# dmar-bonn/ipp-rl

Hardware: AMD Instinct MI355X
Metric: env-steps/s (batched) on 50x50 grid (higher is better)
Workload: dtype f32

## Files before the change

ipp-rl_amd/csrc/ipp_common.h:

```cpp
#pragma once
#include <hip/hip_runtime.h>
#include <stdint.h>
#include <type_traits>

#include "../../include/ipp_engine.h"

#include "ipp_instrument.h"

namespace ipp {

constexpr int kWave = 64;
constexpr int kCountSlots = 64;
#ifndef IPP_PREP_THREADS
#define IPP_PREP_THREADS 128
#endif
constexpr int kPrepThreads = IPP_PREP_THREADS;
constexpr int kMaxTileThreads = 640;
constexpr int kBandRows = 20;
constexpr double kSqrt3 = 1.7320508075688772;

struct ItemHdr {
    int env, dst, rank, status;
    int xl, xr, yu, yd;
    int w, h, nx, ny;
// ... 88 lines not shown
    float* mean;
    float* diag;
    float* gt;
    int* gt_slot;
    double* prior;
    int* rank;
    int* colspan;
    int* colrect;
    int rect_meta;
    int patch;
    int pw, ph;
    int pstride;
    int plw;
    int pcap;
    int punits;
    int pos0;
    unsigned long long* counters;
    unsigned long long* item_counts;
    float* cov;
    uint64_t cov_slot;
    ItemHdr* hdr;
    float* linv;
    float* yv;
    float* q;
    float* wc;
    double* partial;
    double* dbg;
    int dbg_capture;
    double* grf_h;
    double2* grf_cs;
// ... 338 lines not shown
```

ipp-rl_amd/csrc/ipp_engine.hip:

```cpp
#include <hip/hip_runtime.h>
#include <hip/hip_ext.h>

#include <algorithm>
#include <cmath>
#include <cstdarg>
#include <cstdio>
#include <cstdlib>
#include <cstring>
#include <new>
#include <string>
#include <vector>

#include "ipp_common.h"
#include "ipp_host.h"
#include "k_gain.h"
#include "k_gain_factor.h"
#include "k_step_factor.h"
#include "k_step_patch.h"
#include "k_gain_wave.h"
#include "k_misc.h"
#include "k_grf_dft.h"
#include "k_grf_hartley.h"
#include "k_grf_fft.h"
#include "k_fields.h"
// ... 70 lines not shown
    size_t tree_step_lds = 0;
    size_t tree_gain_lds = 0;
    hipStream_t side = nullptr;
    hipEvent_t ev_begin = nullptr, ev_end = nullptr;
    hipEvent_t ev_prep[8] = {};
    ProfSlot prof[kProfKinds];
    std::vector<ProfEvent> prof_pending;
    int last_n = 0;
    uint64_t last_needed_bytes = 0;
};

struct Layout {
    int N, Npad, T, n_tiles, win_tiles, MC, FC, QS, q_rows, VEC;
    bool patch;
    PatchGeo pg;
    uint64_t off_mean, off_diag, off_gt, off_gtslot, off_prior, off_rank, off_span, off_cnt, off_icnt, off_cov, off_hdr, off_linv, off_yv, off_q, off_wc,
        off_partial, off_dbg, off_grfh, off_grfcs, off_grfg, off_grfhp, off_grfamp, off_grfraw, off_grfraw2, off_sc_hdr, off_sc_ext, off_sc_mask, off_sc_G, off_sc_P, off_tr_cov, off_tr_diag, off_tr_meta, off_sc_ndiag, total, cov_slot_floats;
};

uint64_t q_item_floats(const Layout& L) {
    const uint64_t lq = ((uint64_t)L.MC * L.MC + L.MC + 3) & ~(uint64_t)3;
    uint64_t q = lq + (uint64_t)(L.q_rows + 8) * L.QS;
    if (L.patch) q = std::max<uint64_t>(q, (uint64_t)L.q_rows * kPatchRec);
    return (q + 15) & ~(uint64_t)15;
}

bool patch_layout(const ipp_config& c, int MC, const Switches& sw) {
    if (c.state_repr != IPP_FACTOR || c.window_rows <= 0 || MC != 9) return false;
    if (c.tile_threads != 0) return false;
    if (c.x_dim % 2 != 0 || c.x_dim > 256 || c.y_dim > 256) return false;
    if (!(c.x_dim > 2 * c.window_rows + 13)) return false;
// ... 89 lines not shown
        const long rows = std::min<long>(c.y_dim, 2L * c.window_rows + 2L * L.MC);
        L.win_tiles = (int)std::min<long>(L.n_tiles, (rows * c.x_dim + 64 * L.VEC - 1) / (64 * L.VEC) + 1);
    }
    L.q_rows = (c.state_repr == IPP_FACTOR) ? c.rank_cap : L.FC;
    L.cov_slot_floats = (c.state_repr == IPP_FACTOR) ? (uint64_t)c.rank_cap * L.Npad : (uint64_t)L.N * L.Npad;
    if (L.patch) L.cov_slot_floats = (uint64_t)c.rank_cap * L.pg.pstride;
    uint64_t o = 0;
    const uint64_t cap = c.capacity, mb = c.max_batch, np = L.Npad;
    L.off_mean = o; o += up(cap * np * 4);
    L.off_diag = o; o += up(cap * np * 4);
    L.off_gt = o; o += up(2 * cap * np * 4);
    L.off_gtslot = o; o += up(2 * cap * 4);
    L.off_prior = o; o += up(cap * 2 * 8);
    L.off_rank = o; o += up(cap * 4);
    L.off_span = o; o += (c.state_repr == IPP_FACTOR) ? up(2 * cap * (uint64_t)c.rank_cap * 4) : 0;
    L.off_cnt = o; o += up((uint64_t)kCountSlots * 128);
    L.off_icnt = o; o += up((uint64_t)c.max_batch * 16);
    L.off_cov = o; o += up(cap * L.cov_slot_floats * 4);
    L.off_hdr = o; o += up(mb * sizeof(ItemHdr));
    L.off_linv = o; o += up(mb * L.MC * L.MC * 4);
    L.off_yv = o; o += up(mb * L.MC * 4);
    L.off_q = o; o += up(mb * q_item_floats(L) * 4 + 4096);
    L.off_wc = o; o += (c.state_repr == IPP_DENSE) ? up(mb * L.MC * np * 4) : 0;
    L.off_partial = o; o += up(mb * L.n_tiles * 8);
    L.off_dbg = o; o += up(mb * (2 * L.MC * L.MC + 2 * L.MC) * 8);
    L.off_grfh = o; o += up((uint64_t)L.N * 8);
    L.off_grfcs = o; o += up((uint64_t)c.x_dim * 16);
    L.off_grfg = o; o += up((uint64_t)(c.y_dim / 2 + 1) * c.x_dim * 8);
    {
        const uint64_t npad = 16 * (uint64_t)((std::max(c.x_dim, c.y_dim) + 15) / 16);
// ... 128 lines not shown
        for (auto& x : iv[k]) {
            if (x.first > end) { p.busy_ms += x.second - x.first; end = x.second; }
            else if (x.second > end) { p.busy_ms += x.second - end; end = x.second; }
        }
        p.busy_launches += (int64_t)iv[k].size();
    }
}

size_t gain_lds_bytes(const View& v, int q_chunk, int lut_cap) {
    const size_t MC = v.meas_cap, QS = v.q_stride;
    size_t b = std::max((size_t)(q_chunk + 2 * kPipe) * QS, (size_t)((lut_cap + 3) & ~3)) * 4 + ((MC * MC + 3) & ~(size_t)3) * 4 + ((MC + 3) & ~(size_t)3) * 4 + 16 * 8;
    b += (size_t)std::max(q_chunk, v.q_rows) * 4;
    return (b + 15) & ~(size_t)15;
}

#define IPP_STEP_PATCH_KERNELS(X)      \
    X(2, kPatchKP, kPatchMinW, 0)      \
    X(3, kPatchKP, kPatchMinW, 0)      \
    X(3, kPatchKP, kPatchMinW, 1)      \
    X(3, kPatchKP, kPatchMinW, 2)      \
    X(2, IPP_PATCH_BIGKP, 6, 0)
#define IPP_TREE_PATCH_KERNELS(X) X(3, 0) X(3, 1)

using StepPatchKernel = decltype(&k_step_patch<3>);
using TreePatchKernel = decltype(&k_tree_patch<3>);
template <bool BUD>
StepPatchKernel patch_kernel(const PatchVariant& pv) {
#define X(NW, KPN, MINW, RJN) \
    if (pv.waves == NW && pv.kpn == KPN && pv.minw == MINW && pv.rjn == RJN) return k_step_patch<NW, KPN, MINW, RJN, BUD>;
    IPP_STEP_PATCH_KERNELS(X)
#undef X
    return nullptr;
}
TreePatchKernel tree_patch_kernel(const PatchVariant& pv) {
#define X(NW, RJN) if (pv.waves == NW && pv.rjn == RJN) return k_tree_patch<NW, RJN>;
    IPP_TREE_PATCH_KERNELS(X)
#undef X
    return nullptr;
}

template <int MC, int VEC>
void launch_chunk(Engine* e, const View& v, const int32_t* env_ids, const int32_t* dst_ids, int n, const double* action,
                  const double* prev, const float* noise, unsigned flags, float* reward, int32_t* status, hipStream_t s,
                  hipEvent_t prep_done, const AutoReset& ar) {
// ... 281 lines not shown
    v.meas_cap = L.MC; v.fp_cap = L.FC; v.q_stride = L.QS; v.q_rows = L.q_rows; v.q_item = q_item_floats(L);
    v.res = cfg->resolution; v.tanx = cfg->tan_half_fov_x; v.tany = cfg->tan_half_fov_y; v.rf_alt = cfg->rf_altitude;
    v.coeff_a = cfg->coeff_a; v.coeff_b = cfg->coeff_b; v.sv0 = cfg->signal_variance; v.ls0 = cfg->length_scale;
    v.ls_max = (cfg->state_repr == IPP_FACTOR && cfg->window_rows > 0 && cfg->window_rows < std::max(cfg->x_dim, cfg->y_dim)) ? max_length_scale(*cfg) : 0.0;
    v.vmax = cfg->max_v; v.amax = cfg->max_a; v.thr = cfg->value_threshold; v.kf = cfg->interval_factor;
    v.prior_kind = kind;
    char* base = reinterpret_cast<char*>(arena);
    v.mean = reinterpret_cast<float*>(base + L.off_mean);
    v.diag = reinterpret_cast<float*>(base + L.off_diag);
    v.gt = reinterpret_cast<float*>(base + L.off_gt);
    v.gt_slot = reinterpret_cast<int*>(base + L.off_gtslot);
    v.prior = reinterpret_cast<double*>(base + L.off_prior);
    v.rank = reinterpret_cast<int*>(base + L.off_rank);
    v.colspan = reinterpret_cast<int*>(base + L.off_span);
    v.colrect = v.colspan + (size_t)cfg->capacity * cfg->rank_cap;
    v.dbg_capture = 0;
    v.counters = reinterpret_cast<unsigned long long*>(base + L.off_cnt);
    v.item_counts = reinterpret_cast<unsigned long long*>(base + L.off_icnt);
    v.window_rows = (cfg->state_repr == IPP_FACTOR) ? std::max(0, cfg->window_rows) : 0;
    v.tile_cells = (cfg->state_repr == IPP_FACTOR && cfg->window_rows > 0) ? 64 * L.VEC : L.T * L.VEC;
    v.tile_shift = -1;
    for (int sh = 0; sh < 20; ++sh) if ((1 << sh) == v.tile_cells) v.tile_shift = sh;
    v.clip_cols = (cfg->state_repr == IPP_FACTOR && cfg->window_rows > 0 && L.T != 64 && cfg->x_dim > 2 * cfg->window_rows + 13) ? 1 : 0;
    const int lut_tile_rows = (v.tile_cells + cfg->x_dim - 1) / cfg->x_dim + 1;
    const bool lut_complete = (size_t)std::min(cfg->y_dim, std::max(0, cfg->window_rows) + lut_tile_rows + 6) * cfg->x_dim <= 12288;
    e->rect_ok = v.clip_cols && L.MC == 9 && L.VEC == 2 && cfg->x_dim % 2 == 0 && lut_complete;
    e->rect_commit = e->rect_ok && 5 * (2 * cfg->window_rows + 7) <= 2 * cfg->x_dim;
    e->rect_tree = v.clip_cols && L.MC == 9 && cfg->x_dim % L.VEC == 0 && lut_complete && 5 * (2 * cfg->window_rows + 5 + 2 * (L.VEC - 1)) <= 2 * cfg->x_dim;
    if (sw.rect_tree) e->rect_tree = v.clip_cols && L.MC == 9 && cfg->x_dim % L.VEC == 0 && lut_complete && *sw.rect_tree != 0;
    if (sw.rect) { e->rect_commit = e->rect_ok && *sw.rect == 2; e->rect_ok = e->rect_ok && *sw.rect != 0; }
// ... 82 lines not shown
            delete e;
            return fail(-1, "gain kernel needs %zu B of LDS (> 160 KiB): lower rank_cap", need);
        }
    }
    if (e->prep_lds > 160 * 1024) {
        delete e;
        return fail(-1, "prologue needs %zu B of LDS (> 160 KiB): lower rank_cap or max_measurements", e->prep_lds);
    }
    const int lds = (int)e->prep_lds;
    (void)hipFuncSetAttribute(reinterpret_cast<const void*>(&k_prepare<9, IPP_FACTOR>), hipFuncAttributeMaxDynamicSharedMemorySize, lds);
    (void)hipFuncSetAttribute(reinterpret_cast<const void*>(&k_prepare<9, IPP_DENSE>), hipFuncAttributeMaxDynamicSharedMemorySize, lds);
    (void)hipFuncSetAttribute(reinterpret_cast<const void*>(&k_prepare<25, IPP_FACTOR>), hipFuncAttributeMaxDynamicSharedMemorySize, lds);
    (void)hipFuncSetAttribute(reinterpret_cast<const void*>(&k_prepare<25, IPP_DENSE>), hipFuncAttributeMaxDynamicSharedMemorySize, lds);
    {
        auto opt_in = [](auto* kernel) { (void)hipFuncSetAttribute(reinterpret_cast<const void*>(kernel), hipFuncAttributeMaxDynamicSharedMemorySize, 160 * 1024); };
#define X(NW, KPN, MINW, RJN) opt_in(k_step_patch<NW, KPN, MINW, RJN, false>); opt_in(k_step_patch<NW, KPN, MINW, RJN, true>);
        IPP_STEP_PATCH_KERNELS(X)
#undef X
#define X(NW, RJN) opt_in(k_tree_patch<NW, RJN>);
        IPP_TREE_PATCH_KERNELS(X)
#undef X
    }
    (void)hipFuncSetAttribute(reinterpret_cast<const void*>(&k_grf_conv<5, true>), hipFuncAttributeMaxDynamicSharedMemorySize, 120 * 1024);
    (void)hipFuncSetAttribute(reinterpret_cast<const void*>(&k_grf_conv<8, true>), hipFuncAttributeMaxDynamicSharedMemorySize, 120 * 1024);
    const int glds = (int)e->gain_lds;
    (void)hipFuncSetAttribute(reinterpret_cast<const void*>(&k_gain<9, 4, IPP_FACTOR>), hipFuncAttributeMaxDynamicSharedMemorySize, glds);
    (void)hipFuncSetAttribute(reinterpret_cast<const void*>(&k_gain<25, 2, IPP_FACTOR>), hipFuncAttributeMaxDynamicSharedMemorySize, glds);
    (void)hipFuncSetAttribute(reinterpret_cast<const void*>(&k_gain_factor<9, 4>), hipFuncAttributeMaxDynamicSharedMemorySize, glds);
    (void)hipFuncSetAttribute(reinterpret_cast<const void*>(&k_step_factor<9, 4>), hipFuncAttributeMaxDynamicSharedMemorySize, glds);
    (void)hipFuncSetAttribute(reinterpret_cast<const void*>(&k_gain_factor<9, 2>), hipFuncAttributeMaxDynamicSharedMemorySize, glds);
    (void)hipFuncSetAttribute(reinterpret_cast<const void*>(&k_step_factor<9, 2>), hipFuncAttributeMaxDynamicSharedMemorySize, glds);
// ... 1043 lines not shown
```

ipp-rl_amd/csrc/k_misc.h:

```cpp
#pragma once
#include "ipp_common.h"

namespace ipp {

struct InitAction { double p[3]; };

__global__ void k_reset_small(View v, const int* __restrict__ env_ids, int n_items,
                              const double* __restrict__ prior_scale, const float* __restrict__ gt_in,
                              double* __restrict__ prev_out, InitAction init) {
    const int item = blockIdx.y;
    if (item >= n_items) return;
    const int env = env_ids ? env_ids[item] : item;
    if (env < 0 || env >= v.cap) return;
    double sv = prior_scale ? prior_scale[2 * item + 0] : v.sv0;
    double ls = prior_scale ? prior_scale[2 * item + 1] : v.ls0;
    if (v.ls_max > 0.0 && ls > v.ls_max * (1.0 + 1e-12)) sv = ls = NAN;
    const int cell = blockIdx.x * blockDim.x + threadIdx.x;
    if (cell == 0) {
        v.rank[env] = 0;
        v.prior[2 * env + 0] = sv;
        v.prior[2 * env + 1] = ls;
        if (prev_out)
            for (int k = 0; k < 3; ++k) prev_out[3 * env + k] = init.p[k];
    }
// ... 174 lines not shown
    if (blockIdx.x == 0) {
        for (int i = threadIdx.x; i < v.Npad; i += blockDim.x) {
            v.mean[(size_t)d * v.Npad + i] = v.mean[(size_t)s * v.Npad + i];
            v.diag[(size_t)d * v.Npad + i] = v.diag[(size_t)s * v.Npad + i];
            gt_plane(v, d)[i] = gt_plane(v, s)[i];
        }
        if (threadIdx.x == 0) {
            v.prior[2 * d + 0] = v.prior[2 * s + 0];
            v.prior[2 * d + 1] = v.prior[2 * s + 1];
        }
        if (v.mode == IPP_FACTOR)
            for (int i = threadIdx.x; i < r; i += blockDim.x)
            {
                v.colspan[(size_t)d * v.rank_cap + i] = v.colspan[(size_t)s * v.rank_cap + i];
                v.colrect[(size_t)d * v.rank_cap + i] = v.colrect[(size_t)s * v.rank_cap + i];
            }
    }
}
__global__ void k_fork_rank(View v, const int* __restrict__ src_ids, const int* __restrict__ dst_ids, int n_items) {
    const int item = blockIdx.x * blockDim.x + threadIdx.x;
    if (item >= n_items) return;
    const int s = src_ids[item], d = dst_ids[item];
    if (s < 0 || s >= v.cap || d < 0 || d >= v.cap) return;
    v.rank[d] = v.rank[s];
}

__global__ __launch_bounds__(256) void k_read_cov_factor(View v, int env, float* __restrict__ out) {
    const int i = blockIdx.y;
    const int j = blockIdx.x * blockDim.x + threadIdx.x;
    if (i >= v.N || j >= v.N) return;
// ... 121 lines not shown
```

ipp-rl_amd/csrc/k_step_patch.h:

```cpp
#pragma once
#include <algorithm>
#include <cstdlib>
#include <type_traits>
#include "ipp_common.h"
#include "k_gain.h"
#include "k_gain_factor.h"
#include "k_prepare.h"

namespace ipp {

constexpr int kPatchRec = 16;
constexpr int kPatchKP = 8;
constexpr int kPatchRowAux = 2;
constexpr int kPatchStoreAux = IPP_NT_STORES ? 2 : 0;
constexpr int kPatchMinW = 6;
constexpr int kPatchWavesDefault = 3;
constexpr int kPatchWavesPerCu = 4 * kPatchMinW;
constexpr int kPatchCtl = 32;
constexpr int kPatchMaxRank = 512;

struct PatchGeo {
    int pw, ph, pstride, plw, punits;
};
inline PatchGeo patch_geometry(int W, int H, int R) {
// ... 88 lines not shown
    if (lane == 0) {
        L.done[item] = done ? 1 : 0;
        if (rs) {
            const long long ep = L.episode[env] + 1;
            L.episode[env] = ep;
            L.budget[env] = budget_start(L, env, ep);
            L.depth[env] = 0;
        } else {
            L.budget[env] = bud - cost;
            L.depth[env] = dep + 1;
        }
        if (flags & IPP_RESET_ON_DONE) L.refill[pos] = rs ? env : -1;
    }
}

template <int NW, int KPN = kPatchKP, int MINW = kPatchMinW, int RJN = 0, bool BUD = false>
__global__ __launch_bounds__(64 * NW, MINW) void k_step_patch(
    View v, const int* __restrict__ env_ids, int n_items, const double* __restrict__ action,
    const double* __restrict__ prev_action, const float* __restrict__ meas_noise, unsigned flags,
    int* __restrict__ status_out, float* __restrict__ reward_out, AutoReset ar) {
    constexpr int MC = 9, VEC = 2, NT = kWave * NW, KP = KPN;
    static_assert(KPN <= kPatchKP, "the row lists are padded for kPatchKP entries");
    static_assert(NW >= 2, "wave 0 runs the m x m algebra, wave 1 the observation");
    constexpr int RJ = RJN > 0 ? RJN : (kPatchMaxRank + NT - 1) / NT;
    constexpr int OW = 1;
    constexpr int TW = (NW > 2) ? 2 : OW;
    extern __shared__ __attribute__((aligned(16))) unsigned char smem_sp[];
    const PatchLds lds(smem_sp, v.pcap, v.plw * v.plw, NW, v.punits, v.rank_cap);
    if ((int)blockIdx.x >= n_items) return;
    const int item = launch_item(v, blockIdx.x, n_items);
    const int tid = threadIdx.x, lane = tid & (kWave - 1), wave = tid / kWave;
    if (tid == 0) IPP_MARK(item, 0);
    IPP_WT_DECL;
    int* next_unit = lds.ctl; int* done_waves = lds.ctl + 1; int* solve_flag = lds.ctl + 2; int* obs_flag = lds.ctl + 3;
    int* wcnt = lds.ctl + 8;

    const int env0 = env_ids ? env_ids[item] : item + v.env_base;
    const bool slots_ok = env0 >= 0 && env0 < v.cap;
    const int envc = slots_ok ? env0 : 0;
    const double ax = action[3 * item + 0], ay = action[3 * item + 1], az = action[3 * item + 2];
    const double px = prev_action[3 * item + 0], py = prev_action[3 * item + 1], pz = prev_action[3 * item + 2];
    const int rank_ld = v.rank[envc];
    const double sv_d = v.prior[2 * envc + 0], ls_d = v.prior[2 * envc + 1];
    const int otid = tid - kWave * OW;
    const float eps_ld = (meas_noise && otid >= 0 && otid < MC) ? meas_noise[(size_t)item * MC + otid] : 0.f;
    double bud_ld = 0.0;
    int dep_ld = 0;
    if constexpr (BUD) { bud_ld = ar.led.budget[envc]; dep_ld = ar.led.depth[envc]; }
    const int* __restrict__ rects = v.colrect + (size_t)envc * v.rank_cap;
    unsigned rc_pre[RJ];
#pragma unroll
    for (int j = 0; j < RJ; ++j) {
        const int k = tid + j * NT;
        rc_pre[j] = (k < v.rank_cap) ? (unsigned)rects[k] : 0u;
    }

    const int R = v.window_rows;
    const PrepLds<MC> pl(lds.small);
    ItemHdr h;
    if (__builtin_amdgcn_readfirstlane(wave) == 0) {
        h = make_item_header<MC, IPP_FACTOR>(v, env0, env0, slots_ok, ax, ay, az, px, py, pz, rank_ld, sv_d, ls_d, flags);
        const int r0 = max(0, h.yu - R), r1 = min(v.H - 1, h.yd + R);
        const int c0 = max(0, h.xl - R) & ~(VEC - 1), c1 = min(v.W - 1, min(v.W - 1, h.xr + R) | (VEC - 1));
        if (h.m > 0 && (r1 - r0 + 1 > v.ph || c1 - c0 + 1 > v.pw)) {
            h.status = IPP_STATUS_BAD_FOOTPRINT; h.m = 0; h.f = 0; h.rows = 0; h.commit = 0;
        }
        if (tid == 0) {
            *pl.hs = h;
            *next_unit = 0; *done_waves = 0; *solve_flag = 0; *obs_flag = 0;
            lds.red[0] = 0.0; lds.red[1] = 0.0;
// ... 37 lines not shown

    ObsRegs oregs;
    {
        const int ly = div_small(max(otid, 0), h.w), lx = max(otid, 0) - ly * h.w;
        oregs.gt = (!cov_only && otid >= 0 && otid < f) ? gt_env[(h.yu + ly) * v.W + h.xl + lx] : 0.f;
        const Block mob = block_of(min(max(otid, 0), m - 1), h.nx, h.rf, h.w, h.h);
#pragma unroll
        for (int a = 0; a < 4; ++a) {
            const int aa = min(a, mob.count() - 1);
            const int cell = (h.yu + mob.y0 + blk_dy(aa, mob.bw)) * v.W + h.xl + mob.x0 + blk_dx(aa, mob.bw);
            oregs.mean[a] = (!cov_only && otid >= 0 && otid < m && a < mob.count()) ? mean_env[cell] : 0.f;
        }
        oregs.eps = eps_ld;
    }

    bool con[RJ];
    unsigned long long bal[RJ];
#pragma unroll
    for (int j = 0; j < RJ; ++j) {
        const int k = tid + j * NT;
        const unsigned rc = rc_pre[j];
        const int r0k = rc & 0xff, r1k = (rc >> 8) & 0xff, c0k = (rc >> 16) & 0xff, c1k = rc >> 24;
        con[j] = k < r && r0k <= h.yd && r1k >= h.yu && c0k <= h.xr && c1k >= h.xl;
        bal[j] = __ballot(con[j]);
        if (lane == 0) wcnt[j * NW + wave] = __popcll(bal[j]);
    }
    const int ttid = tid - kWave * TW;
    if (ttid >= 0 && ttid < MC) {
        const Block bb = block_of(min(ttid, m - 1), h.nx, h.rf, h.w, h.h);
        for (int a = 0; a < 4; ++a) {
            const int aa = min(a, bb.count() - 1);
            const int ly = bb.y0 + blk_dy(aa, bb.bw), lx = bb.x0 + blk_dx(aa, bb.bw);
            lds.fb_yx[4 * ttid + a] = (h.yu + ly) | ((h.xl + lx) << 16);
            lds.fb_w[4 * ttid + a] = (ttid < m && a < bb.count()) ? (float)bb.weight : 0.f;
            if (ttid < m) pl.bfi[4 * ttid + a] = bfi_pack(ly, lx, h.w);
        }
        if (ttid < m) { pl.bcnt[ttid] = bb.count(); pl.bwt[ttid] = bb.weight; }
    }
    __syncthreads();
    if (tid == 0) IPP_MARK(item, 4);
    IPP_EXIT_POINT(2);
    int pos[RJ];
    int n_c = 0;
#pragma unroll
    for (int j = 0; j < RJ; ++j) {
        int before = 0, all = 0;
#pragma unroll
        for (int w = 0; w < NW; ++w) {
            const int c = wcnt[j * NW + w];
            before += (w < wave) ? c : 0;
            all += c;
        }
        pos[j] = n_c + before + __popcll(bal[j] & ((1ull << lane) - 1ull));
        n_c += all;
    }
    unsigned short* klist = lds.ridx;
    unsigned* rclist = reinterpret_cast<unsigned*>(pl.S);
    static_assert(4 * kPatchMaxRank <= (3 * MC * (MC + 1) + 3 * MC + 2 * 4 * MC) * 8, "rectangle list does not fit the fp64 scratch");
#pragma unroll
    for (int j = 0; j < RJ; ++j)
        if (con[j]) { klist[pos[j]] = (unsigned short)(tid + j * NT); rclist[pos[j]] = rc_pre[j]; }
    __syncthreads();
    static_assert(4 * kPatchMaxRank <= (3 * MC * (MC + 1) + 3 * MC + 4 * MC) * 8, "rectangle list reaches pl.ktab");

    const int wave_u = __builtin_amdgcn_readfirstlane(wave);
    auto mine = [&](int i) { return (i % NW) == wave_u; };
    const auto slot_rs = __builtin_amdgcn_make_buffer_rsrc(slot, 0, 0x7ffffff0, 0x00020000);
    const auto row_rs = __builtin_amdgcn_make_buffer_rsrc(slot - v.pstride, 0, 0x7ffffff0, 0x00020000);
    auto gather_issue = [&](unsigned rc, int k, bool on, float (&l)[MC][4]) {
        const unsigned first = on ? (rc & 0x00ff00ffu) : 0xffffffffu;
        const unsigned extent = on ? (((rc >> 8) & 0x00ff00ffu) - (rc & 0x00ff00ffu)) : 0u;
        const int base4 = (k * v.pstride - (int)(rc & 0xff) * pw - (int)((rc >> 16) & 0xff)) * 4;
        typedef unsigned short us2g __attribute__((ext_vector_type(2)));
#pragma unroll
        for (int i = 0; i < MC; ++i) {
#pragma unroll
            for (int a = 0; a < 4; ++a) l[i][a] = 0.f;
            if (i < m && mine(i)) {
                const int cnt = uni(pl.bcnt[i]);
#pragma unroll
                for (int a = 0; a < 4; ++a) {
                    if (a < cnt) {
                        const unsigned yx = (unsigned)uni(lds.fb_yx[4 * i + a]);
                        const int cell4 = (int)((yx & 0xffffu) * (unsigned)pw + (yx >> 16)) * 4;
                        const us2g d = __builtin_bit_cast(us2g, yx) - __builtin_bit_cast(us2g, first);
                        const bool in = __builtin_bit_cast(unsigned, __builtin_elementwise_min(d, __builtin_bit_cast(us2g, extent))) == __builtin_bit_cast(unsigned, d);
                        const unsigned voff = in ? (unsigned)(base4 + cell4) : 0xffffffffu;
                        l[i][a] = __builtin_bit_cast(float, __builtin_amdgcn_raw_buffer_load_b32(slot_rs, voff, 0, 0));
                    }
                }
            }
        }
        __builtin_amdgcn_sched_barrier(0);
    };
    auto gather_store = [&](unsigned rc, int k, bool on, int a_pos, const float (&l)[MC][4]) {
        if (!on) return;
        float* dst = (a_pos < cap) ? lds.rec + (size_t)a_pos * kPatchRec : nullptr;
        float* gdst = (a_pos >= cap) ? ovf + (size_t)(a_pos - cap) * kPatchRec : nullptr;
#pragma unroll
        for (int i = 0; i < MC; ++i) {
            if (i < m && mine(i)) {
                const int cnt = uni(pl.bcnt[i]);
                float t = l[i][0];
                if (cnt > 1) t += l[i][1];
                if (cnt > 2) t += l[i][2] + l[i][3];
                const float val = -(t * lds.fb_w[4 * i]);
                if (dst) dst[i] = val;
                if (gdst) gdst[i] = val;
            }
        }
        if (wave_u != 0) return;
#pragma unroll
        for (int i = 0; i < 12; ++i)
            if (i >= m) {
                if (dst) dst[i] = 0.f;
                if (gdst) gdst[i] = 0.f;
            }
        const int r0k = rc & 0xff, r1k = (rc >> 8) & 0xff, c0k = (rc >> 16) & 0xff, c1k = rc >> 24;
        const int shift = (r0n - r0k) * pw + (c0n - c0k);
        const float4 meta = make_float4(__int_as_float((k * v.pstride + shift + v.pstride) * 4),
                                        __int_as_float(r0k | (c0k << 16)),
                                        __int_as_float((r1k - r0k) | ((c1k - c0k) << 16)),
                                        __int_as_float(k));
        if (dst) reinterpret_cast<float4*>(dst)[3] = meta;
        if (gdst) reinterpret_cast<float4*>(gdst)[3] = meta;
    };
    {
        float l0[MC][4];
        const bool any0 = n_c > 0;
        const bool on0 = lane < n_c;
        const int k0 = on0 ? (int)klist[lane] : 0;
        const unsigned rc0 = on0 ? rclist[lane] : 0u;
        if (any0) gather_issue(rc0, k0, on0, l0);
        {
            const float s3 = prior_scale_f(v.prior_kind, v.res, h.ls);
            const int lw = v.plw;
            with_prior_kind(v.prior_kind, [&](auto kind) {
                for (int i = tid; i < lw * lw; i += NT) {
                    const int dr = div_small(i, lw), dc = i - dr * lw;
                    lds.lut[i] = prior_f<decltype(kind)::value>(dr, dc, s3, h.sv);
                }
            });
            if (ttid >= 0 && ttid < f) { const int ky = div_small(ttid, h.w); pl.ktab[ttid] = prior_d(v.prior_kind, ky, ttid - ky * h.w, v.res, sv_d, ls_d); }
        }
        if (tid == 0) IPP_MARK(item, 5);
        if (any0) gather_store(rc0, k0, on0, lane, l0);
    }
#pragma unroll 1
    for (int t0 = kWave; t0 < n_c; t0 += kWave) {
        const int t = t0 + lane;
        const bool on = t < n_c;
        const int kk = on ? (int)klist[t] : 0;
        const unsigned rc = on ? rclist[t] : 0u;
        float l[MC][4];
        gather_issue(rc, kk, on, l);
        gather_store(rc, kk, on, t, l);
    }
    if ((flags & IPP_UPDATE_PREV) && tid == 0) {
        double* pwr = const_cast<double*>(prev_action);
        pwr[3 * item + 0] = ax; pwr[3 * item + 1] = ay; pwr[3 * item + 2] = az;
    }
    const int n_lds = min(n_c, cap), n_ovf = n_c - n_lds;
    if (n_ovf > 0) asm volatile("s_waitcnt vmcnt(0)" ::: "memory");
    __syncthreads();
    if (tid == 0) IPP_MARK(item, 1);
    IPP_WT(6);
    IPP_EXIT_POINT(3);

    int status_w0 = 0;
    if (wave == 0) {
        status_w0 = solve_wave_fast<MC>(v, h, item, flags, lds.small, lds.rec, 1, kPatchRec, lds.Ls, lds.ys, nullptr, status_out,
                                        obs_flag, n_lds, n_ovf > 0 ? ovf : nullptr, n_ovf);
        __builtin_amdgcn_fence(__ATOMIC_RELEASE, "workgroup");
        if (lane == 0) __hip_atomic_store(solve_flag, status_w0 == IPP_STATUS_NOT_PD ? 2 : 1, __ATOMIC_RELEASE, __HIP_MEMORY_SCOPE_WORKGROUP);
        if (lane == 0) IPP_MARK(item, 7);
    } else if (wave == OW) {
        observe_wave<MC>(v, h, flags, lds.small, oregs);
        __builtin_amdgcn_fence(__ATOMIC_RELEASE, "workgroup");
        if (lane == 0) __hip_atomic_store(obs_flag, 1, __ATOMIC_RELEASE, __HIP_MEMORY_SCOPE_WORKGROUP);
    }
    IPP_WT(7);
    IPP_EXIT_POINT(4);
    const UnitGeo ug = unit_geometry(r0n, c0n, hn, wn);
    const int n_units = ug.n_units;

    const int n_fast = min(n_lds, 2 * kWave);
    unsigned mcofs[2], mlo[2], mex[2];
#pragma unroll
    for (int p2 = 0; p2 < 2; ++p2) {
        const int a = p2 * kWave + lane;
        mcofs[p2] = 0u; mlo[p2] = 0x0000ffffu; mex[p2] = 0u;
// ... 38 lines not shown
    int arrived = 0;
    if (lane == 0) arrived = atomicAdd(done_waves, 1);
    arrived = __builtin_amdgcn_readfirstlane(arrived);
    if (arrived == 0 && lane == 0) IPP_MARK(item, 6);
    if (arrived != NW - 1) { IPP_WT_FLUSH(lane); return; }
    __builtin_amdgcn_fence(__ATOMIC_ACQUIRE, "workgroup");
    dead = __hip_atomic_load(solve_flag, __ATOMIC_ACQUIRE, __HIP_MEMORY_SCOPE_WORKGROUP) == 2;
    const bool commit_item = commit_u && !dead;
    const double cost_d = pl.hs->cost_d;
    const int t_span = pl.hs->t_lo | (pl.hs->t_hi << 16);
    if (lane == 0) {
        IPP_MARK(item, 2);
        double tot = 0.0;
        for (int t = 0; t < n_units; ++t) tot += lds.unit_red[t];
        reward_out[item] = dead ? NAN : (float)(tot / (cost_d + 1.0));
        if (commit_item) v.rank[env_u] = r + m;
        if (cnt[0]) {
            unsigned long long* ic = v.item_counts + 2 * (size_t)item;
            atomicAdd(ic, cnt[0]);
            atomicAdd(ic + 1, cnt[1]);
        }
    }
    if (commit_item && lane < m) {
        v.colspan[(size_t)env_u * v.rank_cap + r + lane] = t_span;
        v.colrect[(size_t)env_u * v.rank_cap + r + lane] = (int)rect_pack(r0n, r1n, c0n, c1n);
    }
    if constexpr (BUD) ledger_close(v, ar, flags, env_u, item, v.pos0 + (int)blockIdx.x, bud_ld, dep_ld, cost_d, lane);
    else if (reset_k >= 0) wave_reset_env(v, ar, env_u, reset_k, lane);
    IPP_WT(8);
    IPP_WT_FLUSH(lane);
}
// ... 22 lines not shown
```

ipp-rl_amd/csrc/patch_launch.h:

```cpp
#pragma once
#include <algorithm>
#include <climits>
#include <cstdlib>
#include <optional>

#include "k_step_patch.h"

#ifndef IPP_PATCH_BIGKP
#define IPP_PATCH_BIGKP 4
#endif

namespace ipp {

inline std::optional<int> env_int(const char* name) { const char* s = getenv(name); return s ? std::optional<int>(atoi(s)) : std::nullopt; }
inline int env_int_in(const char* name, int lo, int hi, int otherwise) { const int x = env_int(name).value_or(otherwise); return x >= lo && x <= hi ? x : otherwise; }
struct Switches {
    std::optional<int> patch = env_int("IPP_PATCH");
    std::optional<int> patch_cap = env_int("IPP_PATCH_CAP");
    int two_min_items = std::max(0, env_int("IPP_PATCH_TWO_MIN").value_or(6144));
    int big_min_items = env_int("IPP_PATCH_BIG").value_or(16384);
    std::optional<int> rect = env_int("IPP_RECT");
    std::optional<int> rect_meta = env_int("IPP_RECT_META");
    std::optional<int> fused = env_int("IPP_FUSED");
    std::optional<int> step_chunks = env_int("IPP_STEP_CHUNKS");
// ... 30 lines not shown
}

inline int staged_records(int records, int rank_cap) { return records >= rank_cap ? rank_cap : (records & ~7); }
inline int lds_share_records(const View& v, int wgs_per_cu, int waves, int min_records, int fallback, int prev_cap = INT_MAX) {
    const size_t rec = kPatchRec * 4;
    size_t budget = (size_t)160 * 1024 / wgs_per_cu / 1280 * 1280;
    budget = std::min(budget, (size_t)13 * 1280);
    const size_t fixed = patch_lds_bytes(v, 0, waves);
    if (fixed + min_records * rec > budget) return std::min(staged_records(fallback, v.rank_cap), prev_cap);
    const int fit = (int)((budget - fixed) / rec);
    return std::min(staged_records(fit - 1, v.rank_cap), prev_cap);
}

inline PatchPlan make_patch_plan(const View& v, const Switches& sw) {
    PatchPlan p = {};
    static_assert(kPatchWavesDefault == 3, "the first tier's RJN counts rounds of 192 threads");
    const int pcap = sw.patch_cap ? staged_records(std::max(8, *sw.patch_cap), v.rank_cap)
                                  : lds_share_records(v, kPatchWavesPerCu / kPatchWavesDefault, kPatchWavesDefault, 17, 16);
    p.tier[p.n_tiers++] = patch_variant(v, 0, kPatchWavesDefault, kPatchKP, kPatchMinW, v.rank_cap <= 192 ? 1 : v.rank_cap <= 384 ? 2 : 0, pcap);
    if (!sw.patch_cap && sw.two_min_items > 0) {
        p.two_wave_tier = p.n_tiers;
        p.tier[p.n_tiers++] = patch_variant(v, sw.two_min_items, 2, kPatchKP, kPatchMinW, 0, lds_share_records(v, 12, 2, 17, 16, pcap));
    }
    if (p.two_wave_tier && sw.big_min_items > 0) {
        const int pc = lds_share_records(v, 12, 2, 33, 0, p.tier[p.n_tiers - 1].pcap);
        if (pc > 0) p.big_tier = p.n_tiers;
        if (pc > 0) p.tier[p.n_tiers++] = patch_variant(v, sw.big_min_items, 2, IPP_PATCH_BIGKP, 6, 0, pc);
    }
    p.tree = patch_variant(v, 0, kPatchWavesDefault, kPatchKP, kPatchMinW, v.rank_cap <= 192 ? 1 : 0, pcap);
    return p;
}

}
```

Measured before the change: 60.82 million.

## Scan per-step rectangle table per wave instead of per-rank rect ballots

Adds a per-environment step table that records, for each committed step, the rank range and the bounding rectangle. The patch step kernel then tests rectangles per step within a single wave and expands the hits into a per-wave row list, replacing the per-rank rectangle test across all threads with its cross-wave count exchange and two block barriers. The block-geometry reads become register readlanes instead of LDS loads, and each wave keeps only its own measurement rows. In exchange it adds a global table write at commit time and a copy of the table on env cloning, and the rank-count template variants are removed.

```diff
diff --git a/ipp-rl_amd/csrc/ipp_common.h b/ipp-rl_amd/csrc/ipp_common.h
--- a/ipp-rl_amd/csrc/ipp_common.h
+++ b/ipp-rl_amd/csrc/ipp_common.h
@@ -126,6 +126,7 @@
     int plw;
     int pcap;
     int punits;
+    uint2* steptab;
     int pos0;
     unsigned long long* counters;
     unsigned long long* item_counts;
diff --git a/ipp-rl_amd/csrc/ipp_engine.hip b/ipp-rl_amd/csrc/ipp_engine.hip
--- a/ipp-rl_amd/csrc/ipp_engine.hip
+++ b/ipp-rl_amd/csrc/ipp_engine.hip
@@ -108,7 +108,7 @@
     int N, Npad, T, n_tiles, win_tiles, MC, FC, QS, q_rows, VEC;
     bool patch;
     PatchGeo pg;
-    uint64_t off_mean, off_diag, off_gt, off_gtslot, off_prior, off_rank, off_span, off_cnt, off_icnt, off_cov, off_hdr, off_linv, off_yv, off_q, off_wc,
+    uint64_t off_mean, off_diag, off_gt, off_gtslot, off_prior, off_rank, off_span, off_steptab, off_cnt, off_icnt, off_cov, off_hdr, off_linv, off_yv, off_q, off_wc,
         off_partial, off_dbg, off_grfh, off_grfcs, off_grfg, off_grfhp, off_grfamp, off_grfraw, off_grfraw2, off_sc_hdr, off_sc_ext, off_sc_mask, off_sc_G, off_sc_P, off_tr_cov, off_tr_diag, off_tr_meta, off_sc_ndiag, total, cov_slot_floats;
 };
 
@@ -228,6 +228,7 @@
     L.off_prior = o; o += up(cap * 2 * 8);
     L.off_rank = o; o += up(cap * 4);
     L.off_span = o; o += (c.state_repr == IPP_FACTOR) ? up(2 * cap * (uint64_t)c.rank_cap * 4) : 0;
+    L.off_steptab = o; o += L.patch ? up(cap * (uint64_t)c.rank_cap * 8) : 0;
     L.off_cnt = o; o += up((uint64_t)kCountSlots * 128);
     L.off_icnt = o; o += up((uint64_t)c.max_batch * 16);
     L.off_cov = o; o += up(cap * L.cov_slot_floats * 4);
@@ -386,20 +387,18 @@
     return (b + 15) & ~(size_t)15;
 }
 
-#define IPP_STEP_PATCH_KERNELS(X)      \
-    X(2, kPatchKP, kPatchMinW, 0)      \
-    X(3, kPatchKP, kPatchMinW, 0)      \
-    X(3, kPatchKP, kPatchMinW, 1)      \
-    X(3, kPatchKP, kPatchMinW, 2)      \
-    X(2, IPP_PATCH_BIGKP, 6, 0)
+#define IPP_STEP_PATCH_KERNELS(X)   \
+    X(2, kPatchKP, kPatchMinW)      \
+    X(3, kPatchKP, kPatchMinW)      \
+    X(2, IPP_PATCH_BIGKP, 6)
 #define IPP_TREE_PATCH_KERNELS(X) X(3, 0) X(3, 1)
 
 using StepPatchKernel = decltype(&k_step_patch<3>);
 using TreePatchKernel = decltype(&k_tree_patch<3>);
 template <bool BUD>
 StepPatchKernel patch_kernel(const PatchVariant& pv) {
-#define X(NW, KPN, MINW, RJN) \
-    if (pv.waves == NW && pv.kpn == KPN && pv.minw == MINW && pv.rjn == RJN) return k_step_patch<NW, KPN, MINW, RJN, BUD>;
+#define X(NW, KPN, MINW) \
+    if (pv.waves == NW && pv.kpn == KPN && pv.minw == MINW) return k_step_patch<NW, KPN, MINW, BUD>;
     IPP_STEP_PATCH_KERNELS(X)
 #undef X
     return nullptr;
@@ -711,6 +710,7 @@
     v.rank = reinterpret_cast<int*>(base + L.off_rank);
     v.colspan = reinterpret_cast<int*>(base + L.off_span);
     v.colrect = v.colspan + (size_t)cfg->capacity * cfg->rank_cap;
+    v.steptab = L.patch ? reinterpret_cast<uint2*>(base + L.off_steptab) : nullptr;
     v.dbg_capture = 0;
     v.counters = reinterpret_cast<unsigned long long*>(base + L.off_cnt);
     v.item_counts = reinterpret_cast<unsigned long long*>(base + L.off_icnt);
@@ -823,7 +823,7 @@
     (void)hipFuncSetAttribute(reinterpret_cast<const void*>(&k_prepare<25, IPP_DENSE>), hipFuncAttributeMaxDynamicSharedMemorySize, lds);
     {
         auto opt_in = [](auto* kernel) { (void)hipFuncSetAttribute(reinterpret_cast<const void*>(kernel), hipFuncAttributeMaxDynamicSharedMemorySize, 160 * 1024); };
-#define X(NW, KPN, MINW, RJN) opt_in(k_step_patch<NW, KPN, MINW, RJN, false>); opt_in(k_step_patch<NW, KPN, MINW, RJN, true>);
+#define X(NW, KPN, MINW) opt_in(k_step_patch<NW, KPN, MINW, false>); opt_in(k_step_patch<NW, KPN, MINW, true>);
         IPP_STEP_PATCH_KERNELS(X)
 #undef X
 #define X(NW, RJN) opt_in(k_tree_patch<NW, RJN>);
diff --git a/ipp-rl_amd/csrc/k_misc.h b/ipp-rl_amd/csrc/k_misc.h
--- a/ipp-rl_amd/csrc/k_misc.h
+++ b/ipp-rl_amd/csrc/k_misc.h
@@ -212,6 +212,7 @@
             {
                 v.colspan[(size_t)d * v.rank_cap + i] = v.colspan[(size_t)s * v.rank_cap + i];
                 v.colrect[(size_t)d * v.rank_cap + i] = v.colrect[(size_t)s * v.rank_cap + i];
+                if (v.patch) v.steptab[(size_t)d * v.rank_cap + i] = v.steptab[(size_t)s * v.rank_cap + i];
             }
     }
 }
diff --git a/ipp-rl_amd/csrc/k_step_patch.h b/ipp-rl_amd/csrc/k_step_patch.h
--- a/ipp-rl_amd/csrc/k_step_patch.h
+++ b/ipp-rl_amd/csrc/k_step_patch.h
@@ -126,7 +126,7 @@
     }
 }
 
-template <int NW, int KPN = kPatchKP, int MINW = kPatchMinW, int RJN = 0, bool BUD = false>
+template <int NW, int KPN = kPatchKP, int MINW = kPatchMinW, bool BUD = false>
 __global__ __launch_bounds__(64 * NW, MINW) void k_step_patch(
     View v, const int* __restrict__ env_ids, int n_items, const double* __restrict__ action,
     const double* __restrict__ prev_action, const float* __restrict__ meas_noise, unsigned flags,
@@ -134,7 +134,6 @@
     constexpr int MC = 9, VEC = 2, NT = kWave * NW, KP = KPN;
     static_assert(KPN <= kPatchKP, "the row lists are padded for kPatchKP entries");
     static_assert(NW >= 2, "wave 0 runs the m x m algebra, wave 1 the observation");
-    constexpr int RJ = RJN > 0 ? RJN : (kPatchMaxRank + NT - 1) / NT;
     constexpr int OW = 1;
     constexpr int TW = (NW > 2) ? 2 : OW;
     extern __shared__ __attribute__((aligned(16))) unsigned char smem_sp[];
@@ -145,7 +144,6 @@
     if (tid == 0) IPP_MARK(item, 0);
     IPP_WT_DECL;
     int* next_unit = lds.ctl; int* done_waves = lds.ctl + 1; int* solve_flag = lds.ctl + 2; int* obs_flag = lds.ctl + 3;
-    int* wcnt = lds.ctl + 8;
 
     const int env0 = env_ids ? env_ids[item] : item + v.env_base;
     const bool slots_ok = env0 >= 0 && env0 < v.cap;
@@ -159,13 +157,8 @@
     double bud_ld = 0.0;
     int dep_ld = 0;
     if constexpr (BUD) { bud_ld = ar.led.budget[envc]; dep_ld = ar.led.depth[envc]; }
-    const int* __restrict__ rects = v.colrect + (size_t)envc * v.rank_cap;
-    unsigned rc_pre[RJ];
-#pragma unroll
-    for (int j = 0; j < RJ; ++j) {
-        const int k = tid + j * NT;
-        rc_pre[j] = (k < v.rank_cap) ? (unsigned)rects[k] : 0u;
-    }
+    const uint2* __restrict__ stab = v.steptab + (size_t)envc * v.rank_cap;
+    const uint2 st_pre = (lane < v.rank_cap) ? stab[lane] : make_uint2(0u, 0u);
 
     const int R = v.window_rows;
     const PrepLds<MC> pl(lds.small);
@@ -233,97 +226,110 @@
         oregs.eps = eps_ld;
     }
 
-    bool con[RJ];
-    unsigned long long bal[RJ];
-#pragma unroll
-    for (int j = 0; j < RJ; ++j) {
-        const int k = tid + j * NT;
-        const unsigned rc = rc_pre[j];
+    const int wave_u = __builtin_amdgcn_readfirstlane(wave);
+    const int ttid = tid - kWave * TW;
+    const Block bb = block_of(min(lane, m - 1), h.nx, h.rf, h.w, h.h);
+    const int bcn = bb.count();
+    const float bwf = (float)bb.weight;
+    int byx[4];
+#pragma unroll
+    for (int a = 0; a < 4; ++a) {
+        const int aa = min(a, bcn - 1);
+        const int ly = bb.y0 + blk_dy(aa, bb.bw), lx = bb.x0 + blk_dx(aa, bb.bw);
+        byx[a] = (h.yu + ly) | ((h.xl + lx) << 16);
+        if (wave_u == TW && lane < MC) {
+            lds.fb_yx[4 * lane + a] = byx[a];
+            lds.fb_w[4 * lane + a] = (lane < m && a < bcn) ? bwf : 0.f;
+            if (lane < m) pl.bfi[4 * lane + a] = bfi_pack(ly, lx, h.w);
+        }
+    }
+    if (wave_u == TW && lane < m) { pl.bcnt[lane] = bcn; pl.bwt[lane] = bb.weight; }
+
+    unsigned short* wlist = lds.ridx + (size_t)wave_u * (v.rank_cap + KP);
+    int n_c = 0;
+    int n_steps = 0;
+    int kend = 0;
+    bool more = false;
+    int s_d = 0;
+    unsigned s_rc = 0u;
+    auto scan_round = [&](const uint2 st) {
+        const int k0 = st.x & 0xffffu, mm = st.x >> 16, end = k0 + mm;
+        int prev = __shfl_up(end, 1, kWave);
+        if (lane == 0) prev = kend;
+        const bool ok = mm >= 1 && mm <= MC && k0 == prev && end <= r;
+        const unsigned long long bad = __ballot(!ok);
+        const int nv = bad ? (int)__builtin_ctzll(bad) : kWave;
+        const unsigned rc = st.y;
         const int r0k = rc & 0xff, r1k = (rc >> 8) & 0xff, c0k = (rc >> 16) & 0xff, c1k = rc >> 24;
-        con[j] = k < r && r0k <= h.yd && r1k >= h.yu && c0k <= h.xr && c1k >= h.xl;
-        bal[j] = __ballot(con[j]);
-        if (lane == 0) wcnt[j * NW + wave] = __popcll(bal[j]);
-    }
-    const int ttid = tid - kWave * TW;
-    if (ttid >= 0 && ttid < MC) {
-        const Block bb = block_of(min(ttid, m - 1), h.nx, h.rf, h.w, h.h);
-        for (int a = 0; a < 4; ++a) {
-            const int aa = min(a, bb.count() - 1);
-            const int ly = bb.y0 + blk_dy(aa, bb.bw), lx = bb.x0 + blk_dx(aa, bb.bw);
-            lds.fb_yx[4 * ttid + a] = (h.yu + ly) | ((h.xl + lx) << 16);
-            lds.fb_w[4 * ttid + a] = (ttid < m && a < bb.count()) ? (float)bb.weight : 0.f;
-            if (ttid < m) pl.bfi[4 * ttid + a] = bfi_pack(ly, lx, h.w);
-        }
-        if (ttid < m) { pl.bcnt[ttid] = bb.count(); pl.bwt[ttid] = bb.weight; }
-    }
-    __syncthreads();
+        const bool con = lane < nv && r0k <= h.yd && r1k >= h.yu && c0k <= h.xr && c1k >= h.xl;
+        const int cm = con ? mm : 0;
+        int p0 = 0, tot = 0;
+#pragma unroll
+        for (int b = 0; b < 4; ++b) {
+            const unsigned long long bl = __ballot(((cm >> b) & 1) != 0);
+            p0 += (int)__builtin_amdgcn_mbcnt_hi((unsigned)(bl >> 32), __builtin_amdgcn_mbcnt_lo((unsigned)bl, 0u)) << b;
+            tot += __popcll(bl) << b;
+        }
+#pragma unroll
+        for (int j = 0; j < MC; ++j)
+            if (j < cm) wlist[p0 + j] = (unsigned short)lane;
+        __builtin_amdgcn_wave_barrier();
+        s_d = k0 - p0;
+        s_rc = rc;
+        if (nv > 0) kend = __builtin_amdgcn_readlane(end, nv - 1);
+        n_steps += nv;
+        more = nv == kWave && kend < r;
+        return tot;
+    };
+    int n_round = scan_round(st_pre);
+    int* step_slot = lds.ctl + 8;
     if (tid == 0) IPP_MARK(item, 4);
     IPP_EXIT_POINT(2);
-    int pos[RJ];
-    int n_c = 0;
-#pragma unroll
-    for (int j = 0; j < RJ; ++j) {
-        int before = 0, all = 0;
-#pragma unroll
-        for (int w = 0; w < NW; ++w) {
-            const int c = wcnt[j * NW + w];
-            before += (w < wave) ? c : 0;
-            all += c;
-        }
-        pos[j] = n_c + before + __popcll(bal[j] & ((1ull << lane) - 1ull));
-        n_c += all;
-    }
-    unsigned short* klist = lds.ridx;
-    unsigned* rclist = reinterpret_cast<unsigned*>(pl.S);
-    static_assert(4 * kPatchMaxRank <= (3 * MC * (MC + 1) + 3 * MC + 2 * 4 * MC) * 8, "rectangle list does not fit the fp64 scratch");
-#pragma unroll
-    for (int j = 0; j < RJ; ++j)
-        if (con[j]) { klist[pos[j]] = (unsigned short)(tid + j * NT); rclist[pos[j]] = rc_pre[j]; }
-    __syncthreads();
-    static_assert(4 * kPatchMaxRank <= (3 * MC * (MC + 1) + 3 * MC + 4 * MC) * 8, "rectangle list reaches pl.ktab");
-
-    const int wave_u = __builtin_amdgcn_readfirstlane(wave);
-    auto mine = [&](int i) { return (i % NW) == wave_u; };
+
+
     const auto slot_rs = __builtin_amdgcn_make_buffer_rsrc(slot, 0, 0x7ffffff0, 0x00020000);
     const auto row_rs = __builtin_amdgcn_make_buffer_rsrc(slot - v.pstride, 0, 0x7ffffff0, 0x00020000);
-    auto gather_issue = [&](unsigned rc, int k, bool on, float (&l)[MC][4]) {
+    constexpr int NB = (MC + NW - 1) / NW;
+    auto gather_issue = [&](unsigned rc, int k, bool on, float (&l)[NB][4]) {
         const unsigned first = on ? (rc & 0x00ff00ffu) : 0xffffffffu;
         const unsigned extent = on ? (((rc >> 8) & 0x00ff00ffu) - (rc & 0x00ff00ffu)) : 0u;
         const int base4 = (k * v.pstride - (int)(rc & 0xff) * pw - (int)((rc >> 16) & 0xff)) * 4;
         typedef unsigned short us2g __attribute__((ext_vector_type(2)));
 #pragma unroll
-        for (int i = 0; i < MC; ++i) {
-#pragma unroll
-            for (int a = 0; a < 4; ++a) l[i][a] = 0.f;
-            if (i < m && mine(i)) {
-                const int cnt = uni(pl.bcnt[i]);
+        for (int ii = 0; ii < NB; ++ii) {
+            const int i = wave_u + ii * NW;
+#pragma unroll
+            for (int a = 0; a < 4; ++a) l[ii][a] = 0.f;
+            if (i < m) {
+                const int cnt = __builtin_amdgcn_readlane(bcn, i);
 #pragma unroll
                 for (int a = 0; a < 4; ++a) {
                     if (a < cnt) {
-                        const unsigned yx = (unsigned)uni(lds.fb_yx[4 * i + a]);
+                        const unsigned yx = (unsigned)__builtin_amdgcn_readlane(byx[a], i);
                         const int cell4 = (int)((yx & 0xffffu) * (unsigned)pw + (yx >> 16)) * 4;
                         const us2g d = __builtin_bit_cast(us2g, yx) - __builtin_bit_cast(us2g, first);
                         const bool in = __builtin_bit_cast(unsigned, __builtin_elementwise_min(d, __builtin_bit_cast(us2g, extent))) == __builtin_bit_cast(unsigned, d);
                         const unsigned voff = in ? (unsigned)(base4 + cell4) : 0xffffffffu;
-                        l[i][a] = __builtin_bit_cast(float, __builtin_amdgcn_raw_buffer_load_b32(slot_rs, voff, 0, 0));
+                        l[ii][a] = __builtin_bit_cast(float, __builtin_amdgcn_raw_buffer_load_b32(slot_rs, voff, 0, 0));
                     }
                 }
             }
         }
         __builtin_amdgcn_sched_barrier(0);
     };
-    auto gather_store = [&](unsigned rc, int k, bool on, int a_pos, const float (&l)[MC][4]) {
+    auto gather_store = [&](unsigned rc, int k, bool on, int a_pos, const float (&l)[NB][4]) {
         if (!on) return;
         float* dst = (a_pos < cap) ? lds.rec + (size_t)a_pos * kPatchRec : nullptr;
         float* gdst = (a_pos >= cap) ? ovf + (size_t)(a_pos - cap) * kPatchRec : nullptr;
 #pragma unroll
-        for (int i = 0; i < MC; ++i) {
-            if (i < m && mine(i)) {
-                const int cnt = uni(pl.bcnt[i]);
-                float t = l[i][0];
-                if (cnt > 1) t += l[i][1];
-                if (cnt > 2) t += l[i][2] + l[i][3];
-                const float val = -(t * lds.fb_w[4 * i]);
+        for (int ii = 0; ii < NB; ++ii) {
+            const int i = wave_u + ii * NW;
+            if (i < m) {
+                const int cnt = __builtin_amdgcn_readlane(bcn, i);
+                float t = l[ii][0];
+                if (cnt > 1) t += l[ii][1];
+                if (cnt > 2) t += l[ii][2] + l[ii][3];
+                const float val = -(t * __int_as_float(__builtin_amdgcn_readlane(__float_as_int(bwf), i)));
                 if (dst) dst[i] = val;
                 if (gdst) gdst[i] = val;
             }
@@ -344,12 +350,20 @@
         if (dst) reinterpret_cast<float4*>(dst)[3] = meta;
         if (gdst) reinterpret_cast<float4*>(gdst)[3] = meta;
     };
+    auto take = [&](int t0, bool& on, int& kk, unsigned& rc) {
+        const int t = t0 + lane;
+        on = t < n_round;
+        const int sl = on ? (int)wlist[t] : 0;
+        const int d = __shfl(s_d, sl, kWave);
+        const unsigned rcs = (unsigned)__shfl((int)s_rc, sl, kWave);
+        kk = on ? d + t : 0;
+        rc = on ? rcs : 0u;
+    };
     {
-        float l0[MC][4];
-        const bool any0 = n_c > 0;
-        const bool on0 = lane < n_c;
-        const int k0 = on0 ? (int)klist[lane] : 0;
-        const unsigned rc0 = on0 ? rclist[lane] : 0u;
+        float l0[NB][4];
+        const bool any0 = n_round > 0;
+        bool on0; int k0; unsigned rc0;
+        take(0, on0, k0, rc0);
         if (any0) gather_issue(rc0, k0, on0, l0);
         {
             const float s3 = prior_scale_f(v.prior_kind, v.res, h.ls);
@@ -366,19 +380,25 @@
         if (any0) gather_store(rc0, k0, on0, lane, l0);
     }
 #pragma unroll 1
-    for (int t0 = kWave; t0 < n_c; t0 += kWave) {
-        const int t = t0 + lane;
-        const bool on = t < n_c;
-        const int kk = on ? (int)klist[t] : 0;
-        const unsigned rc = on ? rclist[t] : 0u;
-        float l[MC][4];
-        gather_issue(rc, kk, on, l);
-        gather_store(rc, kk, on, t, l);
+    for (int sbase = 0;;) {
+#pragma unroll 1
+        for (int t0 = (sbase == 0) ? kWave : 0; t0 < n_round; t0 += kWave) {
+            bool on; int kk; unsigned rc;
+            take(t0, on, kk, rc);
+            float l[NB][4];
+            gather_issue(rc, kk, on, l);
+            gather_store(rc, kk, on, n_c + t0 + lane, l);
+        }
+        n_c += n_round;
+        if (!more) break;
+        sbase += kWave;
+        n_round = scan_round((sbase + lane < v.rank_cap) ? stab[sbase + lane] : make_uint2(0u, 0u));
     }
     if ((flags & IPP_UPDATE_PREV) && tid == 0) {
         double* pwr = const_cast<double*>(prev_action);
         pwr[3 * item + 0] = ax; pwr[3 * item + 1] = ay; pwr[3 * item + 2] = az;
     }
+    if (tid == 0) *step_slot = n_steps;
     const int n_lds = min(n_c, cap), n_ovf = n_c - n_lds;
     if (n_ovf > 0) asm volatile("s_waitcnt vmcnt(0)" ::: "memory");
     __syncthreads();
@@ -394,6 +414,9 @@
         if (lane == 0) __hip_atomic_store(solve_flag, status_w0 == IPP_STATUS_NOT_PD ? 2 : 1, __ATOMIC_RELEASE, __HIP_MEMORY_SCOPE_WORKGROUP);
         if (lane == 0) IPP_MARK(item, 7);
     } else if (wave == OW) {
+        asm volatile("" : "+v"(oregs.gt), "+v"(oregs.eps));
+#pragma unroll
+        for (int a = 0; a < 4; ++a) asm volatile("" : "+v"(oregs.mean[a]));
         observe_wave<MC>(v, h, flags, lds.small, oregs);
         __builtin_amdgcn_fence(__ATOMIC_RELEASE, "workgroup");
         if (lane == 0) __hip_atomic_store(obs_flag, 1, __ATOMIC_RELEASE, __HIP_MEMORY_SCOPE_WORKGROUP);
@@ -462,7 +485,10 @@
         double tot = 0.0;
         for (int t = 0; t < n_units; ++t) tot += lds.unit_red[t];
         reward_out[item] = dead ? NAN : (float)(tot / (cost_d + 1.0));
-        if (commit_item) v.rank[env_u] = r + m;
+        if (commit_item) {
+            v.steptab[(size_t)env_u * v.rank_cap + *step_slot] = make_uint2((unsigned)r | ((unsigned)m << 16), rect_pack(r0n, r1n, c0n, c1n));
+            v.rank[env_u] = r + m;
+        }
         if (cnt[0]) {
             unsigned long long* ic = v.item_counts + 2 * (size_t)item;
             atomicAdd(ic, cnt[0]);
diff --git a/ipp-rl_amd/csrc/patch_launch.h b/ipp-rl_amd/csrc/patch_launch.h
--- a/ipp-rl_amd/csrc/patch_launch.h
+++ b/ipp-rl_amd/csrc/patch_launch.h
@@ -68,10 +68,10 @@
 
 inline PatchPlan make_patch_plan(const View& v, const Switches& sw) {
     PatchPlan p = {};
-    static_assert(kPatchWavesDefault == 3, "the first tier's RJN counts rounds of 192 threads");
+    static_assert(kPatchWavesDefault == 3, "the tree kernel's RJN counts rounds of 192 threads");
     const int pcap = sw.patch_cap ? staged_records(std::max(8, *sw.patch_cap), v.rank_cap)
                                   : lds_share_records(v, kPatchWavesPerCu / kPatchWavesDefault, kPatchWavesDefault, 17, 16);
-    p.tier[p.n_tiers++] = patch_variant(v, 0, kPatchWavesDefault, kPatchKP, kPatchMinW, v.rank_cap <= 192 ? 1 : v.rank_cap <= 384 ? 2 : 0, pcap);
+    p.tier[p.n_tiers++] = patch_variant(v, 0, kPatchWavesDefault, kPatchKP, kPatchMinW, 0, pcap);
     if (!sw.patch_cap && sw.two_min_items > 0) {
         p.two_wave_tier = p.n_tiers;
         p.tier[p.n_tiers++] = patch_variant(v, sw.two_min_items, 2, kPatchKP, kPatchMinW, 0, lds_share_records(v, 12, 2, 17, 16, pcap));
```

Result: faster. 62.01 million (median of 6 runs) (+2.0%).
